# KubiakJakub01/Blokus-RL

Hardware: AMD Instinct MI355X
Metric: MCTS sims/sec on 20x20 Blokus (4 players, 256 games/GPU, 100 sims/move) (higher is better)
Workload: dtype fp32 net (fp32 operands split into f16 hi+lo, 3 f16 MFMA products, f32 accumulation: fp32-class error, tests/test_leafnet_gpu.py) / f64 search / u32 bitboards; 1 GPU; config 3 (N=1) / 4 (N=8): AlphaZero self-play 20x20, 256 concurrent games per GPU, 100 sims/move, ResNet-5x64 leaf eval; global_batch=256, parallelism=dp1 (independent games), model=resnet

## Files before the change

### blokus_rl_amd/csrc/mcts.hip

```cpp
#define BK_BOARD_SYNC() ::bk::wave_lds_sync()
#ifdef BK_STAMPS
#include <hip/hip_runtime.h>
static __device__ unsigned long long g_step_stamps[4096][16];
#define BK_MASK_STAMP(i) \
  do { if (threadIdx.x == 0 && blockIdx.x < 4096 && blockDim.x > 256) g_step_stamps[blockIdx.x][i] = __builtin_amdgcn_s_memtime(); } while (0)
#endif
#include <algorithm>
#include <cmath>
#include <cstring>
#include <vector>

#include "../../include/blokus_engine.h"
#include "ctx.h"
#include "legal_rows.h"
#include "mcts_dev.h"

namespace bk {

constexpr int kResetBlocks = 8;
__global__ __launch_bounds__(256) void k_reset(DevMcts m, const int32_t* flags) {
  const int t = blockIdx.y;
  if (flags && !flags[t]) return;
  TabEntry* tab = m.tab + (size_t)t * m.TS;
  for (int i = blockIdx.x * 256 + threadIdx.x; i < m.TS; i += kResetBlocks * 256) tab[i] = TabEntry{0ull, 0u, 0};
  if (blockIdx.x == 0 && threadIdx.x == 0) { m.tree_nodes[t] = 0; m.tree_children[t] = 0; }
}

constexpr int kSelectWaves = 4;
__global__ __launch_bounds__(64 * kSelectWaves) void k_select(DevPreset dp, DevMcts m, const uint32_t* __restrict__ roots,
                                                              const int32_t* __restrict__ active, double cpuct,
                                                              int32_t* __restrict__ status_out, float* __restrict__ obs,
                                                              uint64_t* __restrict__ mask_out, double root_eps, int t0) {
  extern __shared__ __attribute__((aligned(16))) uint32_t lds[];
  __shared__ int status_sh;
  const int t = t0 + blockIdx.x;
  const int wave = __builtin_amdgcn_readfirstlane(threadIdx.x >> 6);
  if (wave == 0) {
    const int st = select_descend(dp, m, t, roots, active, cpuct, status_out, lds, 0, nullptr, root_eps);
    if (lane_id() == 0) status_sh = st;
  }
  __syncthreads();
  select_leaf<kSelectWaves>(dp, m, t, status_sh, obs, mask_out, lds, wave);
}

constexpr int kLeafR = 1;
__global__ __launch_bounds__(256) void k_leaf_logits(DevPreset dp, DevMcts m, const float* __restrict__ feat,
                                                     int64_t ldf, int F, const float* __restrict__ W,
                                                     const float* __restrict__ bias) {
  extern __shared__ __attribute__((aligned(16))) uint32_t lds[];
  leaf_logits_tree<kLeafR>(dp, m, blockIdx.x, blockIdx.y, kLeafBlocks, feat, ldf, F, W, bias, lds);
}

__global__ __launch_bounds__(64) void k_expand_backup(DevPreset dp, DevMcts m, const float* __restrict__ logp,
                                                      const float* __restrict__ values, int prior_mode) {
  extern __shared__ __attribute__((aligned(16))) uint32_t lds[];
  expand_tree(dp, m, blockIdx.x, logp, values, prior_mode, lds);
}

__device__ __forceinline__ void wg_store_handoff() {
  __builtin_amdgcn_s_waitcnt(0x0F70);
  __syncthreads();
  asm volatile("buffer_inv sc0" ::: "memory");
}
constexpr int kStepWaves = 16;
__device__ __forceinline__ void leaf_zero_logits_tree(const DevPreset& dp, const DevMcts& m, int t,
                                                      const float* __restrict__ feat, int64_t ldf, int F,
                                                      uint32_t* lds) {
  const int K = leaf_logits_prologue(dp, m, t, 0, feat, ldf, F, lds);
  if (K < 0 || K > kLeafCap) return;
  const int32_t* ids = reinterpret_cast<const int32_t*>(lds + dp.W32pad);
  for (int j = threadIdx.x; j < K; j += blockDim.x) {
    m.leaf_ids[(size_t)t * kLeafCap + j] = ids[j];
    m.leaf_logit[(size_t)t * kLeafCap + j] = 0.0f;
  }
}
template <bool ROWS>
__device__ __forceinline__ void leaf_step_body(const DevPreset& dp, const DevMcts& m, const int t,
                                               const float* __restrict__ feat, int64_t ldf, int F,
                                               const float* __restrict__ W, const float* __restrict__ bias,
                                               const float* __restrict__ values, int do_select,
                                               const uint32_t* __restrict__ roots,
                                               const int32_t* __restrict__ active, double cpuct,
                                               int32_t* __restrict__ status_out, float* __restrict__ obs,
                                               uint64_t* __restrict__ mask_out, bool uninformed, int root_row) {
  extern __shared__ __attribute__((aligned(16))) uint32_t lds[];
  __shared__ int status_sh;
  const int wave = __builtin_amdgcn_readfirstlane(threadIdx.x >> 6);
#ifdef BK_STAMPS
#define BK_STEP_STAMP(i) \
  do { if (do_select && threadIdx.x == 0 && t < 4096) g_step_stamps[t][i] = __builtin_amdgcn_s_memtime(); } while (0)
#else
#define BK_STEP_STAMP(i) do { } while (0)
#endif
  BK_STEP_STAMP(0);
  if (ROWS && uninformed)
    leaf_zero_logits_tree(dp, m, t, feat, ldf, F, lds);
  else
    leaf_logits_tree<kLeafR>(dp, m, t, 0, 1, feat, ldf, F, W, bias, lds);
  wg_store_handoff();
  BK_STEP_STAMP(1);
  if (wave == 0) expand_tree<ROWS>(dp, m, t, nullptr, values, 2, lds);
  wg_store_handoff();
  BK_STEP_STAMP(2);
  if (!do_select) return;
  if (wave == 0) {
    const int st = select_descend<ROWS>(dp, m, t, roots, active, cpuct, status_out, lds, 0, nullptr, 1e-6, root_row);
    if (lane_id() == 0) status_sh = st;
  }
  __syncthreads();
  BK_STEP_STAMP(3);
  select_leaf<kStepWaves>(dp, m, t, status_sh, obs, mask_out, lds, wave);
  BK_STEP_STAMP(4);
#undef BK_STEP_STAMP
}
__global__ __launch_bounds__(64 * kStepWaves) void k_leaf_step(DevPreset dp, DevMcts m, const float* __restrict__ feat,
                                                                 int64_t ldf, int F, const float* __restrict__ W,
                                                                 const float* __restrict__ bias,
                                                                 const float* __restrict__ values, int do_select,
                                                                 const uint32_t* __restrict__ roots,
                                                                 const int32_t* __restrict__ active, double cpuct,
                                                                 int32_t* __restrict__ status_out,
                                                                 float* __restrict__ obs,
                                                                 uint64_t* __restrict__ mask_out, int t0) {
  leaf_step_body<false>(dp, m, t0 + blockIdx.x, feat, ldf, F, W, bias, values, do_select, roots, active, cpuct,
                        status_out, obs, mask_out, false, -1);
}

template <bool ROWS>
__device__ __forceinline__ void leaf_step_ov_body(const DevPreset& dp, const DevMcts& m, const int t,
                                                  const float* __restrict__ feat, int64_t ldf, int F,
                                                  const float* __restrict__ W, const float* __restrict__ bias,
                                                  const float* __restrict__ values, int do_select,
                                                  const uint32_t* __restrict__ roots,
                                                  const int32_t* __restrict__ active, double cpuct,
                                                  int32_t* __restrict__ status_out, float* __restrict__ obs,
                                                  uint64_t* __restrict__ mask_out, int sel_off, int skipz,
                                                  bool uninformed, int root_row) {
  extern __shared__ __attribute__((aligned(16))) uint32_t lds[];
  __shared__ int status_sh, status0_sh;
  __shared__ StepExpand sx;
  const int wave = __builtin_amdgcn_readfirstlane(threadIdx.x >> 6);
#ifdef BK_STAMPS
#define BK_OV_STAMP(i) \
  do { if (lane_id() == 0 && do_select && t < 4096) g_step_stamps[t][i] = __builtin_amdgcn_s_memtime(); } while (0)
#else
#define BK_OV_STAMP(i) do { } while (0)
#endif
  if (threadIdx.x == 0) {
    sx.ready = 0;
    sx.pready = 0;
    sx.done = 0;
    sx.leaf_ready = 0;
    sx.slice = 0;
    sx.loaded = 0;
    sx.counted = 0;
    sx.written = 0;
    sx.kready = 0;
    sx.hready = 0;
    status_sh = 0;
    status0_sh = m.leaf_status[t];
  }
  if (wave == 0) BK_OV_STAMP(0);
  LeafPre pre{0ull, 0.0f, false};
  if (wave > 0) pre = leaf_pre_load<kStepWaves - 1>(dp, m, t, feat, ldf, F);
  __syncthreads();
  const int status0 = status0_sh;
  int K = -1;
  if (wave > 0) {
    K = leaf_logits_prologue_w<kStepWaves - 1>(dp, m, t, feat, ldf, F, lds, wave, &sx, status0, &pre);
    if (wave == 1 && K >= 0) {
      wait_flag_acquire(&sx.hready);
      StepHead h;
      h.status = sx.hd_status;
      h.node = sx.hd_node;
      h.used = sx.hd_used;
      h.key = sx.hd_key;
      expand_head(m, t, h, K, &sx);
      BK_OV_STAMP(1);
    }
  }
  const int32_t* ids = reinterpret_cast<const int32_t*>(lds + dp.W32pad);
  float* lg = reinterpret_cast<float*>(lds + dp.W32pad + kLeafCap + F);
  uint32_t* lsel = lds + sel_off;
  uint32_t* m32 = lsel + kStateWords + 2 * kMaxN;
  if (wave == 0) {
    const StepHead h = backup_first<ROWS>(m, t, dp.P, values, status0);
    if (h.status == 1) {
      if (lane_id() == 0) {
        sx.hd_status = h.status;
        sx.hd_node = h.node;
        sx.hd_used = h.used;
        sx.hd_key = h.key;
        __hip_atomic_store(&sx.hready, 1, __ATOMIC_RELEASE, __HIP_MEMORY_SCOPE_WORKGROUP);
      }
    } else if (lane_id() == 0) {
      sx.err = -1;
      __hip_atomic_store(&sx.ready, 1, __ATOMIC_RELEASE, __HIP_MEMORY_SCOPE_WORKGROUP);
    }
    BK_OV_STAMP(2);
    if (do_select) {
      __builtin_amdgcn_s_waitcnt(0x0F70);
      asm volatile("buffer_inv sc0" ::: "memory");
      int* pend[3];
      pend[0] = &sx.ready;
      pend[1] = &sx.pready;
      pend[2] = &sx.err;
      const int st = select_descend<ROWS>(dp, m, t, roots, active, cpuct, status_out, lsel, h.key,
                                          h.status == 1 ? pend : nullptr, 1e-6, root_row);
      if (st == 1)
        for (int i = lane_id(); i < dp.W32pad / 4; i += kWave) reinterpret_cast<uint4*>(m32)[i] = make_uint4(0u, 0u, 0u, 0u);
      if (lane_id() == 0) {
        status_sh = st;
        __hip_atomic_store(&sx.leaf_ready, 1, __ATOMIC_RELEASE, __HIP_MEMORY_SCOPE_WORKGROUP);
      }
      BK_OV_STAMP(3);
      leaf_obs_rows<1>(dp, m, t, st, obs, lsel, lane_id());
    }
  }
  if (wave > 0 && K >= 0 && K <= kLeafCap) {
    if (ROWS && uninformed) {
      for (int j = (wave - 1) * kWave + lane_id(); j < K; j += (kStepWaves - 1) * kWave) lg[j] = 0.0f;
    } else {
      leaf_logits_dots<kLeafR>(dp, 0, K, wave - 1, kStepWaves - 1, W, bias, F, lds, nullptr, lg, skipz);
    }
    int done = 0;
    if (lane_id() == 0) done = __hip_atomic_fetch_add(&sx.done, 1, __ATOMIC_ACQ_REL, __HIP_MEMORY_SCOPE_WORKGROUP);
    done = readlane_i(done, 0);
    if (done == kStepWaves - 2) {
      BK_OV_STAMP(4);
      while (__hip_atomic_load(&sx.ready, __ATOMIC_ACQUIRE, __HIP_MEMORY_SCOPE_WORKGROUP) == 0)
        __builtin_amdgcn_s_sleep(1);
      const int err = readlane_i(sx.err, 0);
      if (err == 0) expand_children_lds(m, (int64_t)sx.off, K, ids, lg);
      BK_OV_STAMP(9);
      const bool descended = readlane_i(__hip_atomic_load(&sx.leaf_ready, __ATOMIC_RELAXED,
                                                          __HIP_MEMORY_SCOPE_WORKGROUP), 0) != 0;
      if (!descended) {
        __builtin_amdgcn_s_waitcnt(0x0F70);
        if (lane_id() == 0) __hip_atomic_store(&sx.pready, 1, __ATOMIC_RELEASE, __HIP_MEMORY_SCOPE_WORKGROUP);
      } else if (lane_id() == 0) {
        __hip_atomic_store(&sx.pready, 1, __ATOMIC_RELAXED, __HIP_MEMORY_SCOPE_WORKGROUP);
      }
      BK_OV_STAMP(5);
    }
  }
  if (do_select) {
    while (__hip_atomic_load(&sx.leaf_ready, __ATOMIC_ACQUIRE, __HIP_MEMORY_SCOPE_WORKGROUP) == 0)
      __builtin_amdgcn_s_sleep(1);
    if (readlane_i(status_sh, 0) == 1) mask_slices_claim(dp, lsel, m32, &sx.slice);
    if (wave == 0) BK_OV_STAMP(8);
  }
  __syncthreads();
  if (wave == 0) BK_OV_STAMP(6);
  if (!do_select) return;
  select_leaf<kStepWaves, true, false>(dp, m, t, status_sh, obs, mask_out, lsel, wave);
  if (wave == 0) BK_OV_STAMP(7);
#undef BK_OV_STAMP
}
__global__ __launch_bounds__(64 * kStepWaves) void k_leaf_step_ov(DevPreset dp, DevMcts m, const float* __restrict__ feat,
                                                                    int64_t ldf, int F, const float* __restrict__ W,
                                                                    const float* __restrict__ bias,
                                                                    const float* __restrict__ values, int do_select,
                                                                    const uint32_t* __restrict__ roots,
                                                                    const int32_t* __restrict__ active, double cpuct,
                                                                    int32_t* __restrict__ status_out,
                                                                    float* __restrict__ obs,
                                                                    uint64_t* __restrict__ mask_out, int sel_off,
                                                                    int skipz, int t0) {
  leaf_step_ov_body<false>(dp, m, t0 + blockIdx.x, feat, ldf, F, W, bias, values, do_select, roots, active, cpuct,
                           status_out, obs, mask_out, sel_off, skipz, false, -1);
}

struct RowTabs {
  const int32_t *tree, *net, *sims;
};
struct RowHeads {
  const float* W[BK_ARENA_MAX_NETS];
  const float* bias[BK_ARENA_MAX_NETS];
  int n;
};
__device__ __forceinline__ int row_live_tree(const RowTabs& rows, int r, int sim, int& budget) {
  const int t = __builtin_amdgcn_readfirstlane(rows.tree[r]);
  budget = 0;
  if (t < 0) return -1;
  budget = __builtin_amdgcn_readfirstlane(rows.sims[r]);
  return sim < budget ? t : -1;
}
__device__ __forceinline__ bool row_head(const RowTabs& rows, const RowHeads& hd, int r, const float*& W,
                                         const float*& bias, bool& uninformed) {
  const int k = __builtin_amdgcn_readfirstlane(rows.net[r]);
  uninformed = k < 0;
  W = k == 0 ? hd.W[0] : k == 1 ? hd.W[1] : k == 2 ? hd.W[2] : k == 3 ? hd.W[3] : nullptr;
  bias = k == 0 ? hd.bias[0] : k == 1 ? hd.bias[1] : k == 2 ? hd.bias[2] : k == 3 ? hd.bias[3] : nullptr;
  return k < hd.n;
}

__global__ __launch_bounds__(64 * kSelectWaves) void k_select_rows(DevPreset dp, DevMcts m, RowTabs rows,
                                                                   const uint32_t* __restrict__ roots, double cpuct,
                                                                   int32_t* __restrict__ status_out) {
  extern __shared__ __attribute__((aligned(16))) uint32_t lds[];
  __shared__ int status_sh;
  int budget;
  const int t = row_live_tree(rows, blockIdx.x, 0, budget);
  if (t < 0 || t >= m.T) return;
  const int wave = __builtin_amdgcn_readfirstlane(threadIdx.x >> 6);
  if (wave == 0) {
    const int st = select_descend<true>(dp, m, t, roots, nullptr, cpuct, status_out, lds, 0, nullptr, 1e-6, (int)blockIdx.x);
    if (lane_id() == 0) status_sh = st;
  }
  __syncthreads();
  select_leaf<kSelectWaves>(dp, m, t, status_sh, nullptr, nullptr, lds, wave);
}

__global__ __launch_bounds__(64 * kStepWaves) void k_leaf_step_rows(DevPreset dp, DevMcts m, RowTabs rows, int sim,
                                                                      const float* __restrict__ feat, int64_t ldf, int F,
                                                                      RowHeads heads, const float* __restrict__ values,
                                                                      int do_select, const uint32_t* __restrict__ roots,
                                                                      double cpuct, int32_t* __restrict__ status_out) {
  int budget;
  const int t = row_live_tree(rows, blockIdx.x, sim, budget);
  if (t < 0 || t >= m.T) return;
  const float *W, *bias;
  bool uninformed;
  if (!row_head(rows, heads, blockIdx.x, W, bias, uninformed)) return;
  leaf_step_body<true>(dp, m, t, feat, ldf, F, W, bias, uninformed ? nullptr : values,
                       do_select && sim + 1 < budget, roots, nullptr, cpuct, status_out, nullptr, nullptr, uninformed,
                       (int)blockIdx.x);
}

__global__ __launch_bounds__(64 * kStepWaves) void k_leaf_step_ov_rows(DevPreset dp, DevMcts m, RowTabs rows, int sim,
                                                                         const float* __restrict__ feat, int64_t ldf,
                                                                         int F, RowHeads heads,
                                                                         const float* __restrict__ values, int do_select,
                                                                         const uint32_t* __restrict__ roots, double cpuct,
                                                                         int32_t* __restrict__ status_out, int sel_off,
                                                                         int skipz) {
  int budget;
  const int t = row_live_tree(rows, blockIdx.x, sim, budget);
  if (t < 0 || t >= m.T) return;
  const float *W, *bias;
  bool uninformed;
  if (!row_head(rows, heads, blockIdx.x, W, bias, uninformed)) return;
  leaf_step_ov_body<true>(dp, m, t, feat, ldf, F, W, bias, uninformed ? nullptr : values,
                          do_select && sim + 1 < budget, roots, nullptr, cpuct, status_out, nullptr, nullptr, sel_off,
                          skipz, uninformed, (int)blockIdx.x);
}

__global__ __launch_bounds__(64) void k_arena_move(DevMcts m, RowTabs rows, const uint32_t* __restrict__ roots,
                                                   int32_t* __restrict__ action) {
  const int r = blockIdx.x, l = lane_id();
  const int t = __builtin_amdgcn_readfirstlane(rows.tree[r]);
  if (t < 0 || t >= m.T) {
    if (l == 0) action[r] = -1;
    return;
  }
  const uint64_t key = table_key(roots + (size_t)r * kStateWords);
  int64_t off;
  int K;
  if (!table_find(m, t, key, off, K, nullptr)) {
    if (l == 0) {
      action[r] = -1;
      atomicOr(&m.counters[kCtrErr], (unsigned long long)kErrMissingRoot);
    }
    return;
  }
  double best = -1.0;
  int bi = 0x7fffffff;
  for (int i = l; i < K; i += kWave) {
    const double v = (double)m.ch_N[off + i];
    if (v > best) { best = v; bi = i; }
  }
  wave_argmax(best, bi);
  if (l == 0) action[r] = K > 0 ? m.ch_id[off + bi] : -1;
}

__device__ __forceinline__ double raise_visits(uint32_t n, double e) {
  if (e == 1.0 || n <= 1u) return (double)n;
  return pow((double)n, e);
}

__global__ __launch_bounds__(64) void k_root(DevMcts m, const uint32_t* __restrict__ roots,
                                             const int32_t* __restrict__ active, double temperature, int mode,
                                             int32_t* ids, double* pi, uint32_t* n_out, double* q_out, float* p_out,
                                             int cap, int32_t* counts) {
  const int t = blockIdx.x;
  const int l = lane_id();
  if (active && !active[t]) {
    if (l == 0) counts[t] = 0;
    return;
  }
  const uint32_t* s = roots + (size_t)t * kStateWords;
  const uint64_t key = table_key(s);
  int64_t off;
  int K;
  if (!table_find(m, t, key, off, K, nullptr)) {
    if (l == 0) { counts[t] = -1; atomicOr(&m.counters[kCtrErr], (unsigned long long)kErrMissingRoot); }
    return;
  }
  if (l == 0) counts[t] = K <= cap ? K : -K;
  const int Kc = K <= cap ? K : cap;
  if (mode == 1) {
    for (int i = l; i < Kc; i += kWave) {
      ids[(size_t)t * cap + i] = m.ch_id[off + i];
      n_out[(size_t)t * cap + i] = m.ch_N[off + i];
      q_out[(size_t)t * cap + i] = m.ch_Q[off + i];
      p_out[(size_t)t * cap + i] = m.ch_P[off + i];
    }
    return;
  }
  for (int i = l; i < Kc; i += kWave) ids[(size_t)t * cap + i] = m.ch_id[off + i];
  double* o = pi + (size_t)t * cap;
  if (temperature == 0.0) {
    double best = -1.0;
    int bi = 0x7fffffff;
    for (int i = l; i < K; i += kWave) {
      const double v = (double)m.ch_N[off + i];
      if (v > best) { best = v; bi = i; }
    }
    wave_argmax(best, bi);
    for (int i = l; i < Kc; i += kWave) o[i] = i == bi ? 1.0 : 0.0;
    return;
  }
  constexpr int kRootLds = 2048;
  __shared__ double vals[kRootLds];
  __shared__ double total_sh;
  const double e = 1.0 / temperature;
  for (int i = l; i < K && i < kRootLds; i += kWave) vals[i] = raise_visits(m.ch_N[off + i], e);
  __syncthreads();
  if (l == 0) {
    double total = 0.0;
#pragma unroll 8
    for (int i = 0; i < K; ++i) total += i < kRootLds ? vals[i] : raise_visits(m.ch_N[off + i], e);
    total_sh = total;
  }
  __syncthreads();
  const double total = total_sh;
  for (int i = l; i < Kc; i += kWave) {
    const double v = i < kRootLds ? vals[i] : raise_visits(m.ch_N[off + i], e);
    o[i] = total == 0.0 ? 1.0 / (double)K : v / total;
  }
}

}

using namespace bk;

template <typename T>
static int mcts_alloc(bk_mcts* m, T** p, size_t count) {
  void* q = nullptr;
  int rc = hip_check(hipMalloc(&q, sizeof(T) * (count ? count : 1)), "hipMalloc mcts");
  if (rc) return rc;
  m->allocs.push_back(q);
  *p = (T*)q;
  return BK_OK;
}

extern "C" {

#ifdef BK_STAMPS
int bk_debug_stamps(unsigned long long* out) {
  return hip_check(hipMemcpyFromSymbol(out, HIP_SYMBOL(g_stamps), sizeof(g_stamps)), "stamps");
}
int bk_debug_mask_stamps(unsigned long long* out) {
  return hip_check(hipMemcpyFromSymbol(out, HIP_SYMBOL(g_mask_stamps), sizeof(g_mask_stamps)), "mask stamps");
}
int bk_debug_step_stamps(unsigned long long* out) {
  return hip_check(hipMemcpyFromSymbol(out, HIP_SYMBOL(g_step_stamps), sizeof(g_step_stamps)), "step stamps");
}
#endif

int bk_mcts_create(bk_ctx* ctx, int trees, int node_cap, int64_t child_cap, bk_mcts** out) {
  BK_REQUIRE(ctx && out && trees > 0 && node_cap > 0 && child_cap >= trees, "bad argument");
  BK_REQUIRE(child_cap / trees <= (int64_t)0xffffffff, "bk_mcts_create: child_cap / trees must fit 32 bits");
  BK_REQUIRE(ctx->d_items, "host-only context (created with device < 0)");
  *out = nullptr;
  bk_mcts* m = new bk_mcts();
  m->ctx = ctx;
  DevMcts& d = m->d;
  d.T = trees;
  d.node_cap = node_cap;
  int TS = 64;
  while (TS < 2 * node_cap) TS <<= 1;
  d.TS = TS;
  d.child_cap_per_tree = child_cap / trees;
  const size_t T = (size_t)trees;
  const int W64 = ctx->dp.W64;
  int rc = hip_check(hipSetDevice(ctx->device), "hipSetDevice");
  if (!rc) {
    const size_t C0 = (size_t)d.child_cap_per_tree * T;
    const size_t need = T * TS * sizeof(TabEntry) + C0 * (4 + 4 + 8 + 4) +
                        T * (kMaxDepth * 12 + kStateWords * 4 + kMaxP * 8 + W64 * 8 + kLeafCap * 8 + 64 + 64);
    size_t free_b = 0, total_b = 0;
    if (hipMemGetInfo(&free_b, &total_b) == hipSuccess && need > free_b) {
      delete m;
      char msg[256];
      snprintf(msg, sizeof msg,
               "bk_mcts_create: %d trees x node_cap %d (child_cap %lld) need %.2f GB of device memory, %.2f GB free",
               trees, node_cap, (long long)child_cap, need / 1e9, free_b / 1e9);
      bk::set_error(msg);
      return BK_ENOMEM;
    }
  }
  if (!rc) rc = mcts_alloc(m, &d.tab, T * TS);
  if (!rc) rc = mcts_alloc(m, &d.tree_nodes, T);
  if (!rc) rc = mcts_alloc(m, &d.tree_children, T);
  const size_t C = (size_t)d.child_cap_per_tree * T;
  if (!rc) rc = mcts_alloc(m, &d.ch_id, C);
  if (!rc) rc = mcts_alloc(m, &d.ch_N, C);
  if (!rc) rc = mcts_alloc(m, &d.ch_Q, C);
  if (!rc) rc = mcts_alloc(m, &d.ch_P, C);
  if (!rc) rc = mcts_alloc(m, &d.path_child, T * kMaxDepth);
  if (!rc) rc = mcts_alloc(m, &d.path_pl, T * kMaxDepth);
  if (!rc) rc = mcts_alloc(m, &d.depth, T);
  if (!rc) rc = mcts_alloc(m, &d.leaf_state, T * kStateWords);
  if (!rc) rc = mcts_alloc(m, &d.leaf_status, T);
  if (!rc) rc = mcts_alloc(m, &d.leaf_scores, T * kMaxP);
  if (!rc) rc = mcts_alloc(m, &d.leaf_mask, T * W64);
  if (!rc) rc = mcts_alloc(m, &d.leaf_ids, T * kLeafCap);
  if (!rc) rc = mcts_alloc(m, &d.leaf_logit, T * kLeafCap);
  if (!rc) rc = mcts_alloc(m, &d.leaf_K, T);
  if (!rc) rc = mcts_alloc(m, &d.counters, 8);
  if (!rc) rc = hip_check(hipMemset(d.counters, 0, 8 * sizeof(unsigned long long)), "memset counters");
  if (!rc) rc = mcts_alloc(m, &d.tree_ctr, T * 8);
  if (!rc) rc = hip_check(hipMemset(d.tree_ctr, 0, T * 8 * sizeof(unsigned long long)), "memset tree counters");
  if (!rc) rc = hip_check(hipMemset(d.leaf_status, 0, T * sizeof(int32_t)), "memset status");
  if (!rc) rc = hip_check(hipMemset(d.depth, 0, T * sizeof(int32_t)), "memset depth");
  if (rc) { bk_mcts_destroy(m); return rc; }
  rc = bk_mcts_reset(m, nullptr, nullptr);
  if (!rc) rc = hip_check(hipDeviceSynchronize(), "sync");
  if (rc) { bk_mcts_destroy(m); return rc; }
  *out = m;
  return BK_OK;
}

int bk_mcts_destroy(bk_mcts* m) {
  if (!m) return BK_OK;
  for (void* p : m->allocs) (void)hipFree(p);
  for (hipStream_t s : m->pipe_stream)
    if (s) (void)hipStreamDestroy(s);
  for (hipEvent_t e : m->pipe_step)
    if (e) (void)hipEventDestroy(e);
  for (hipEvent_t e : m->pipe_join)
    if (e) (void)hipEventDestroy(e);
  if (m->pipe_fork) (void)hipEventDestroy(m->pipe_fork);
  delete m;
  return BK_OK;
}

int bk_mcts_reset(bk_mcts* m, const int32_t* reset_flags, void* stream) {
  BK_REQUIRE(m, "null mcts");
  hipLaunchKernelGGL(k_reset, dim3(kResetBlocks, m->d.T), dim3(256), 0, (hipStream_t)stream, m->d,
                     reset_flags);
  return launch_check("k_reset");
// ... 358 lines not shown
```

### blokus_rl_amd/csrc/mcts_dev.h

```cpp
#pragma once
#include <cmath>
#include <vector>

#include "../../include/blokus_engine.h"
#include "ctx.h"
#include "legal_rows.h"

namespace bk {

constexpr int kMaxDepth = 96;
constexpr int kExpandLdsIds = 2048;
constexpr int kGatherRegs = 16;
constexpr int kLeafCap = 2048;
constexpr int kLeafBlocks = 4;
constexpr int kMaxFeat = 2048;
constexpr int kLeafQ = 16;

#ifdef BK_STAMPS
static __device__ unsigned long long g_stamps[2][4096][8];
#define BK_STAMP(k, i) \
  do { if (lane_id() == 0 && blockIdx.x < 4096) g_stamps[k][blockIdx.x][i] = __builtin_amdgcn_s_memtime(); } while (0)
#else
#define BK_STAMP(k, i) do { } while (0)
#endif
// ... 363 lines not shown
  __syncthreads();
  const int wave = threadIdx.x >> 6, l = threadIdx.x & 63;
  if (wave == 0) {
    const int K = compact_ids(dp, m32, ids, kLeafCap);
    if (l == 0) Ksh = K;
  }
  __syncthreads();
  const int K = Ksh;
  if (c == 0 && threadIdx.x == 0) {
    m.leaf_K[t] = K;
    if (K > kLeafCap) atomicOr(&m.counters[kCtrErr], (unsigned long long)kErrLeafCap);
  }
  return K;
}


__device__ __forceinline__ bool nz4(const float4& x) { return x.x != 0.f || x.y != 0.f || x.z != 0.f || x.w != 0.f; }
__device__ __forceinline__ __amdgpu_buffer_rsrc_t w_rsrc(const float* W, unsigned bytes) {
  const uintptr_t a = (uintptr_t)W;
  const uintptr_t u = ((uintptr_t)(unsigned)__builtin_amdgcn_readfirstlane((int)(a >> 32)) << 32) |
                      (unsigned)__builtin_amdgcn_readfirstlane((int)(unsigned)a);
  return __builtin_amdgcn_make_buffer_rsrc((void*)u, 0, (int)bytes, 0x00020000);
}
__device__ __forceinline__ float4 w_load(__amdgpu_buffer_rsrc_t rs, unsigned off, bool use) {
  using u32x4 = unsigned __attribute__((ext_vector_type(4)));
  const u32x4 v = __builtin_bit_cast(u32x4, __builtin_amdgcn_raw_buffer_load_b128(rs, use ? off : 0xFFFFFFF0u, 0, 0));
  return make_float4(__uint_as_float(v.x), __uint_as_float(v.y), __uint_as_float(v.z), __uint_as_float(v.w));
}
template <bool SKIP = false>
__device__ __forceinline__ float row_dot16(const float4* __restrict__ r, const float4* f4, int F4, int sub,
                                           __amdgpu_buffer_rsrc_t rs, unsigned roff) {
  float a0 = 0.f, a1 = 0.f;
  int q = sub;
  for (; q + 48 < F4; q += 64) {
    const float4 x0 = f4[q], x1 = f4[q + 16], x2 = f4[q + 32], x3 = f4[q + 48];
    float4 w0, w1, w2, w3;
    if (SKIP) {
      w0 = w_load(rs, roff + 16u * q, nz4(x0));
      w1 = w_load(rs, roff + 16u * (q + 16), nz4(x1));
      w2 = w_load(rs, roff + 16u * (q + 32), nz4(x2));
      w3 = w_load(rs, roff + 16u * (q + 48), nz4(x3));
    } else {
      w0 = r[q];
      w1 = r[q + 16];
      w2 = r[q + 32];
      w3 = r[q + 48];
    }
    a0 += w0.x * x0.x + w0.y * x0.y + w0.z * x0.z + w0.w * x0.w;
    a1 += w1.x * x1.x + w1.y * x1.y + w1.z * x1.z + w1.w * x1.w;
    a0 += w2.x * x2.x + w2.y * x2.y + w2.z * x2.z + w2.w * x2.w;
    a1 += w3.x * x3.x + w3.y * x3.y + w3.z * x3.z + w3.w * x3.w;
  }
  for (; q < F4; q += 16) {
    const float4 x0 = f4[q];
    const float4 w0 = SKIP ? w_load(rs, roff + 16u * q, nz4(x0)) : r[q];
    a0 += w0.x * x0.x + w0.y * x0.y + w0.z * x0.z + w0.w * x0.w;
  }
  float a = a0 + a1;
#pragma unroll
  for (int o = 8; o >= 1; o >>= 1) a += __shfl_xor(a, o, 16);
  return a;
}

template <int R = 1>
__device__ __forceinline__ void leaf_logits_dots(const DevPreset& dp, int lo, int hi, int wave, int nw,
                                                 const float* __restrict__ W, const float* __restrict__ bias, int F,
                                                 const uint32_t* lds, int32_t* out_ids, float* out_lg,
                                                 int skipz = 0) {
  const int32_t* ids = reinterpret_cast<const int32_t*>(lds + dp.W32pad);
  const float* f = reinterpret_cast<const float*>(lds + dp.W32pad + kLeafCap);
  const int l = threadIdx.x & 63;
  if (R > 1 && (F & 3) == 0 && F <= 64 * kLeafQ) {
    const int F4 = F >> 2;
    const float4* f4 = reinterpret_cast<const float4*>(f);
    const int sub = l & 15, quad = l >> 4;
    for (int j0 = lo + 4 * R * wave; j0 < hi; j0 += 4 * R * nw) {
      int jr[R], idr[R];
      float4 w[R][kLeafQ];
#pragma unroll
      for (int u = 0; u < R; ++u) {
        jr[u] = j0 + 4 * u + quad;
        idr[u] = ids[jr[u] < hi ? jr[u] : lo];
        const float4* r = reinterpret_cast<const float4*>(W + (size_t)idr[u] * F);
#pragma unroll
        for (int k = 0; k < kLeafQ; ++k) w[u][k] = r[sub + 16 * k < F4 ? sub + 16 * k : F4 - 1];
      }
#pragma unroll
      for (int u = 0; u < R; ++u) {
        float a0 = 0.f, a1 = 0.f;
#pragma unroll
        for (int k = 0; k < kLeafQ; ++k) {
          const int q = sub + 16 * k;
          if (q < F4) {
            const float4 x = f4[q];
            const float d = w[u][k].x * x.x + w[u][k].y * x.y + w[u][k].z * x.z + w[u][k].w * x.w;
            if ((k & 1) && sub + 16 * (k | 3) < F4)
              a1 += d;
            else
              a0 += d;
          }
        }
        float a = a0 + a1;
#pragma unroll
        for (int o = 8; o >= 1; o >>= 1) a += __shfl_xor(a, o, 16);
        if (sub == 0 && jr[u] < hi) {
          if (out_ids) out_ids[jr[u]] = idr[u];
          out_lg[jr[u]] = a + bias[idr[u]];
        }
      }
    }
  } else if ((F & 3) == 0) {
    const int F4 = F >> 2;
    const float4* f4 = reinterpret_cast<const float4*>(f);
    const int sub = l & 15, quad = l >> 4;
    const uint64_t wbytes = (uint64_t)dp.A * (uint64_t)F * 4u;
    const bool sk = skipz && wbytes < 0x7FFFFFF0ull;
    const __amdgpu_buffer_rsrc_t wrs = w_rsrc(W, sk ? (unsigned)wbytes : 0u);
    for (int j0 = lo + 4 * wave; j0 < hi; j0 += 4 * nw) {
      const int j = j0 + quad;
      const bool ok = j < hi;
      const int id = ids[ok ? j : lo];
      const float4* wr = reinterpret_cast<const float4*>(W + (size_t)id * F);
      const float a = sk ? row_dot16<true>(wr, f4, F4, sub, wrs, (unsigned)id * (unsigned)F * 4u)
                            : row_dot16<false>(wr, f4, F4, sub, wrs, 0u);
      if (sub == 0 && ok) {
        if (out_ids) out_ids[j] = id;
        out_lg[j] = a + bias[id];
      }
    }
  } else {
    for (int j = lo + wave; j < hi; j += nw) {
      const int id = ids[j];
      const float* r = W + (size_t)id * F;
      float a = 0.f;
      for (int q = l; q < F; q += kWave) a += r[q] * f[q];
      a = wave_sum_f(a);
      if (l == 0) {
        if (out_ids) out_ids[j] = id;
        out_lg[j] = a + bias[id];
      }
    }
  }
}


template <int R = 1>
__device__ __forceinline__ void leaf_logits_tree(const DevPreset& dp, const DevMcts& m, int t, int c, int nc,
                                                 const float* __restrict__ feat, int64_t ldf, int F,
                                                 const float* __restrict__ W, const float* __restrict__ bias,
                                                 uint32_t* lds) {
  const int K = leaf_logits_prologue(dp, m, t, c, feat, ldf, F, lds);
  if (K < 0 || K > kLeafCap) return;
  const int lo = (int)((int64_t)K * c / nc), hi = (int)((int64_t)K * (c + 1) / nc);
  leaf_logits_dots<R>(dp, lo, hi, (int)(threadIdx.x >> 6), (int)(blockDim.x >> 6), W, bias, F, lds,
                      m.leaf_ids + (size_t)t * kLeafCap, m.leaf_logit + (size_t)t * kLeafCap);
}

template <bool ZV = false>
__device__ __forceinline__ void expand_tree(const DevPreset& dp, const DevMcts& m, int t, const float* __restrict__ logp,
                                            const float* __restrict__ values, int prior_mode, uint32_t* lds) {
  uint32_t* m32 = lds;
  __shared__ double vsh[kMaxP];
  const int l = lane_id();
  const bool sparse = prior_mode == 2;
  const int status = m.leaf_status[t];
  const int depth = m.depth[t];
  const int node = m.tree_nodes[t];
  const int64_t used = m.tree_children[t];
  const int leafK = sparse ? m.leaf_K[t] : 0;
  const uint64_t key = table_key(m.leaf_state + (size_t)t * kStateWords);
  if (status == 0) return;
  BK_STAMP(1, 0);
  const size_t pi = (size_t)t * kMaxDepth + l;
  const bool on_path = l < depth;
  const int64_t pchild = on_path ? m.path_child[pi] : 0;
  const int ppl = on_path ? m.path_pl[pi] : 0;
  if (status == 1) {
    int err = 0;
    const int64_t room = m.child_cap_per_tree - used;
    const int64_t off = (int64_t)t * m.child_cap_per_tree + used;
    int32_t* ids_lds = reinterpret_cast<int32_t*>(m32 + dp.W32pad);
    const int cap_lds = kExpandLdsIds;
    int K;
    bool in_lds;
    BK_STAMP(1, 1);
    if (sparse) {
      K = leafK;
      in_lds = true;
      if (K > kLeafCap) err |= kErrLeafCap;
    } else {
      const uint64_t* lm = m.leaf_mask + (size_t)t * dp.W64;
      for (int j = l; j < dp.W64; j += kWave) {
        const uint64_t w = lm[j];
        m32[2 * j] = (uint32_t)w;
        m32[2 * j + 1] = (uint32_t)(w >> 32);
      }
      BK_BOARD_SYNC();
      K = compact_ids(dp, m32, ids_lds, cap_lds);
      in_lds = K <= cap_lds;
      if (!in_lds)
        K = compact_ids(dp, m32, m.ch_id + off, room > 0 ? (int)(room < 0x7fffffff ? room : 0x7fffffff) : 0);
      BK_BOARD_SYNC();
    }
    BK_STAMP(1, 2);
    if (node >= m.node_cap) err |= kErrTable;
    if (K > room) err |= kErrChildPool;
    const float* lp = sparse ? m.leaf_logit + (size_t)t * kLeafCap : logp + (size_t)t * dp.A;
    const int32_t* cid = sparse ? m.leaf_ids + (size_t)t * kLeafCap : (in_lds ? ids_lds : m.ch_id + off);
    auto logit = [&](int i) { return sparse ? lp[i] : lp[cid[i]]; };
    float x[kGatherRegs];
    int32_t xid[kGatherRegs];
#pragma unroll
    for (int j = 0; j < kGatherRegs; ++j) {
      const int i = l + j * kWave;
      const bool ok = !err && i < K;
      x[j] = ok ? logit(i) : -INFINITY;
      xid[j] = ok && in_lds ? cid[i] : 0;
    }
    int free_slot = -1;
    if (!err) {
      int64_t foff;
      int fK;
      if (table_find(m, t, key, foff, fK, &free_slot) || free_slot < 0) err |= kErrTable;
    }
    BK_STAMP(1, 3);
    if (!err) {
      float mx = -INFINITY;
#pragma unroll
      for (int j = 0; j < kGatherRegs; ++j) mx = fmaxf(mx, x[j]);
      for (int i = l + kGatherRegs * kWave; i < K; i += kWave) mx = fmaxf(mx, logit(i));
      float lse = 0.0f;
      if (prior_mode != 1) {
        mx = wave_max_f(mx);
        float sum = 0.0f;
#pragma unroll
        for (int j = 0; j < kGatherRegs; ++j) sum += l + j * kWave < K ? expf(x[j] - mx) : 0.0f;
        for (int i = l + kGatherRegs * kWave; i < K; i += kWave) sum += expf(logit(i) - mx);
        sum = wave_sum_f(sum);
        lse = logf(sum);
#pragma unroll
        for (int j = 0; j < kGatherRegs; ++j) x[j] = expf((x[j] - mx) - lse);
      }
#pragma unroll
      for (int j = 0; j < kGatherRegs; ++j) {
        const int i = l + j * kWave;
        if (i < K) {
          if (in_lds) m.ch_id[off + i] = xid[j];
          m.ch_N[off + i] = 0u;
          m.ch_Q[off + i] = 0.0;
          m.ch_P[off + i] = x[j];
        }
      }
      for (int i = l + kGatherRegs * kWave; i < K; i += kWave) {
        const float xi = logit(i);
        if (in_lds) m.ch_id[off + i] = cid[i];
        m.ch_N[off + i] = 0u;
        m.ch_Q[off + i] = 0.0;
        m.ch_P[off + i] = prior_mode != 1 ? expf((xi - mx) - lse) : xi;
      }
      if (l == 0) {
        TabEntry e;
        e.key = key;
        e.off = (uint32_t)used;
        e.K = K;
        m.tab[(size_t)t * m.TS + free_slot] = e;
        m.tree_nodes[t] = node + 1;
        m.tree_children[t] = used + K;
        ctr_add(m, t, kCtrExpanded, 1ull);
        ctr_add(m, t, kCtrLeafK, (unsigned long long)K);
      }
    } else if (l == 0) {
      atomicOr(&m.counters[kCtrErr], (unsigned long long)err);
    }
    if (l < dp.P) vsh[l] = ZV && !values ? 0.0 : (double)values[(size_t)t * dp.P + l];
  } else {
    if (l < dp.P) vsh[l] = m.leaf_scores[(size_t)t * kMaxP + l];
  }
  BK_STAMP(1, 4);
  BK_BOARD_SYNC();
  if (on_path) {
    const double v = vsh[ppl];
    const uint32_t n = m.ch_N[pchild];
    const double q = m.ch_Q[pchild];
    m.ch_Q[pchild] = ((double)n * q + v) / (double)(n + 1u);
    m.ch_N[pchild] = n + 1u;
  }
  for (int d = l + kWave; d < depth; d += kWave) {
    const size_t pd = (size_t)t * kMaxDepth + d;
    const int64_t ci = m.path_child[pd];
    const double v = vsh[m.path_pl[pd]];
    const uint32_t n = m.ch_N[ci];
    const double q = m.ch_Q[ci];
    m.ch_Q[ci] = ((double)n * q + v) / (double)(n + 1u);
    m.ch_N[ci] = n + 1u;
  }
  BK_STAMP(1, 5);
}

struct StepExpand {
  long long off;
  int K, err;
  int ready;
  int pready;
  int done;
  int leaf_ready;
  int slice;
  int loaded;
  int counted;
  int written;
  int kready;
  int hready;
  int wcnt[16];
  int hd_status, hd_node;
  long long hd_used;
  unsigned long long hd_key;
};

struct StepHead {
  int status, node;
  int64_t used;
  uint64_t key;
};
template <bool ZV = false>
__device__ __forceinline__ StepHead backup_first(const DevMcts& m, int t, int P, const float* __restrict__ values,
                                                 int status) {
  __shared__ double vsh[kMaxP];
  const int l = lane_id();
  StepHead h;
  h.status = status;
  const int depth = m.depth[t];
  h.node = m.tree_nodes[t];
  h.used = m.tree_children[t];
  h.key = table_key(m.leaf_state + (size_t)t * kStateWords);
  if (h.status == 0) return h;
  const size_t pi = (size_t)t * kMaxDepth + l;
  const bool on_path = l < depth;
  const int64_t pchild = on_path ? m.path_child[pi] : 0;
  const int ppl = on_path ? m.path_pl[pi] : 0;
  if (h.status == 1) {
    if (l < P) vsh[l] = ZV && !values ? 0.0 : (double)values[(size_t)t * P + l];
  } else {
    if (l < P) vsh[l] = m.leaf_scores[(size_t)t * kMaxP + l];
  }
  wave_lds_sync();
  if (on_path) {
    const double v = vsh[ppl];
    const uint32_t n = m.ch_N[pchild];
    const double q = m.ch_Q[pchild];
    m.ch_Q[pchild] = ((double)n * q + v) / (double)(n + 1u);
    m.ch_N[pchild] = n + 1u;
  }
  for (int d = l + kWave; d < depth; d += kWave) {
    const size_t pd = (size_t)t * kMaxDepth + d;
    const int64_t ci = m.path_child[pd];
    const double v = vsh[m.path_pl[pd]];
    const uint32_t n = m.ch_N[ci];
    const double q = m.ch_Q[ci];
    m.ch_Q[ci] = ((double)n * q + v) / (double)(n + 1u);
    m.ch_N[ci] = n + 1u;
  }
  return h;
}

__device__ __forceinline__ void expand_head(const DevMcts& m, int t, const StepHead& h, int K, StepExpand* sx) {
  const int l = lane_id();
  int err = 0;
  if (h.status == 1) {
    const int64_t room = m.child_cap_per_tree - h.used;
    if (K > kLeafCap) err |= kErrLeafCap;
    if (h.node >= m.node_cap) err |= kErrTable;
    if (K > room) err |= kErrChildPool;
    int free_slot = -1;
    if (!err) {
      int64_t foff;
      int fK;
      if (table_find(m, t, h.key, foff, fK, &free_slot) || free_slot < 0) err |= kErrTable;
    }
    if (!err) {
      if (l == 0) {
        TabEntry e;
        e.key = h.key;
        e.off = (uint32_t)h.used;
        e.K = K;
        m.tab[(size_t)t * m.TS + free_slot] = e;
        m.tree_nodes[t] = h.node + 1;
        m.tree_children[t] = h.used + K;
        ctr_add(m, t, kCtrExpanded, 1ull);
        ctr_add(m, t, kCtrLeafK, (unsigned long long)K);
      }
    } else if (l == 0) {
      atomicOr(&m.counters[kCtrErr], (unsigned long long)err);
    }
  }
  __builtin_amdgcn_s_waitcnt(0x0F70);
  if (l == 0) {
    sx->off = (long long)((int64_t)t * m.child_cap_per_tree + h.used);
    sx->K = K;
    sx->err = h.status == 1 ? err : -1;
    __hip_atomic_store(&sx->ready, 1, __ATOMIC_RELEASE, __HIP_MEMORY_SCOPE_WORKGROUP);
  }
}

struct LeafPre {
  uint64_t w;
  float f;
  bool ok;
};
template <int NW>
__device__ __forceinline__ LeafPre leaf_pre_load(const DevPreset& dp, const DevMcts& m, int t,
                                                 const float* __restrict__ feat, int64_t ldf, int F) {
  const int tid = threadIdx.x - kWave, nth = NW * kWave;
  LeafPre p;
  p.ok = dp.W64 <= nth && F <= nth;
  p.w = p.ok && tid < dp.W64 ? m.leaf_mask[(size_t)t * dp.W64 + tid] : 0ull;
  p.f = p.ok && tid < F ? feat[(size_t)t * ldf + tid] : 0.0f;
  return p;
}
template <int NW>
__device__ __forceinline__ int leaf_logits_prologue_w(const DevPreset& dp, const DevMcts& m, int t,
                                                      const float* __restrict__ feat, int64_t ldf, int F,
                                                      uint32_t* lds, int wave, StepExpand* sx, int status,
                                                      const LeafPre* pre = nullptr) {
  uint32_t* m32 = lds;
  int32_t* ids = reinterpret_cast<int32_t*>(lds + dp.W32pad);
  float* f = reinterpret_cast<float*>(lds + dp.W32pad + kLeafCap);
  if (status != 1) return -1;
  const int tid = threadIdx.x - kWave, nth = NW * kWave, l = lane_id();
  if (pre && pre->ok) {
    if (tid < dp.W64) {
      m32[2 * tid] = (uint32_t)pre->w;
      m32[2 * tid + 1] = (uint32_t)(pre->w >> 32);
    }
    if (tid < F) f[tid] = pre->f;
  } else {
    const uint64_t* lm = m.leaf_mask + (size_t)t * dp.W64;
    for (int j = tid; j < dp.W64; j += nth) {
      const uint64_t w = lm[j];
      m32[2 * j] = (uint32_t)w;
      m32[2 * j + 1] = (uint32_t)(w >> 32);
    }
    const float* ft = feat + (size_t)t * ldf;
    for (int i = tid; i < F; i += nth) f[i] = ft[i];
  }
  auto arrive_wait = [&](int* ctr) {
    if (l == 0) __hip_atomic_fetch_add(ctr, 1, __ATOMIC_ACQ_REL, __HIP_MEMORY_SCOPE_WORKGROUP);
    while (__hip_atomic_load(ctr, __ATOMIC_ACQUIRE, __HIP_MEMORY_SCOPE_WORKGROUP) < NW) __builtin_amdgcn_s_sleep(1);
  };
  arrive_wait(&sx->loaded);
  const int w = 64 * (wave - 1) + l;
  uint32_t bits = w < dp.W32 ? m32[w] : 0u;
  const int cnt = __popc(bits);
  const int incl = wave_incl_scan(cnt);
  if (l == kWave - 1) sx->wcnt[wave] = incl;
  arrive_wait(&sx->counted);
  int before = 0, K = 0;
  for (int v = 1; v <= NW; ++v) {
    const int c = sx->wcnt[v];
    before += v < wave ? c : 0;
    K += c;
  }
  int pos = before + incl - cnt;
  while (bits) {
    const int b = __ffs(bits) - 1;
    bits &= bits - 1u;
    if (pos < kLeafCap) ids[pos] = w * 32 + b;
    ++pos;
  }
  arrive_wait(&sx->written);
  if (wave == 1 && l == 0) {
    m.leaf_K[t] = K;
    if (K > kLeafCap) atomicOr(&m.counters[kCtrErr], (unsigned long long)kErrLeafCap);
    __hip_atomic_store(&sx->kready, K + 1, __ATOMIC_RELEASE, __HIP_MEMORY_SCOPE_WORKGROUP);
  }
  return K;
}

#ifdef BK_STAMPS
static __device__ unsigned long long g_mask_stamps[256][16][6];
#endif
__device__ __forceinline__ void mask_slices_claim(const DevPreset& dp, const uint32_t* s, uint32_t* m32, int* counter) {
#ifdef BK_STAMPS
  const unsigned long long t_in = __builtin_amdgcn_s_memtime();
  unsigned long long n_cl = 0, t_max = 0, t_first_claim = 0;
  int last_k = -1;
#endif
  RowCtx c = row_ctx(dp, s, (int)s[kWToMove], m32);
  for (;;) {
#ifdef BK_STAMPS
    const unsigned long long t_s = __builtin_amdgcn_s_memtime();
    if (t_first_claim == 0) t_first_claim = t_s;
#endif
#pragma unroll
    for (int d = 0; d < 5; ++d) asm volatile("" : "+v"(c.fr[d]), "+v"(c.ar[d]));
    asm volatile("" : "+v"(c.r), "+v"(c.rN1), "+v"(c.pieces));
    int k = 0;
    if (lane_id() == 0) k = __hip_atomic_fetch_add(counter, 1, __ATOMIC_RELAXED, __HIP_MEMORY_SCOPE_WORKGROUP);
    k = readlane_i(k, 0);
    if (k >= kMaskWpb) break;
    DevPreset dq = dp;
    asm volatile("" : "+s"(dq.N), "+s"(dq.num_pieces));
    orient_dispatch<kMaskWpb>(dq, c, k, std::make_index_sequence<kMaskWpb>{});
#ifdef BK_STAMPS
    ++n_cl;
    last_k = k;
    const unsigned long long d = __builtin_amdgcn_s_memtime() - t_s;
    t_max = d > t_max ? d : t_max;
#endif
  }
#ifdef BK_STAMPS
  const unsigned long long t_out = __builtin_amdgcn_s_memtime();
  unsigned long long t_warm = 0;
  if (last_k >= 0) {
    DevPreset dq = dp;
    asm volatile("" : "+s"(dq.N), "+s"(dq.num_pieces));
    const unsigned long long t0 = __builtin_amdgcn_s_memtime();
    orient_dispatch<kMaskWpb>(dq, c, last_k, std::make_index_sequence<kMaskWpb>{});
    t_warm = __builtin_amdgcn_s_memtime() - t0;
  }
  const int w = (int)(threadIdx.x >> 6);
  if (lane_id() == 0 && blockIdx.x < 256 && w < 16) {
    g_mask_stamps[blockIdx.x][w][0] = t_in;
    g_mask_stamps[blockIdx.x][w][1] = n_cl;
    g_mask_stamps[blockIdx.x][w][2] = t_out;
    g_mask_stamps[blockIdx.x][w][3] = t_max;
    g_mask_stamps[blockIdx.x][w][4] = t_warm;
    g_mask_stamps[blockIdx.x][w][5] = t_first_claim;
  }
#endif
}

__device__ __forceinline__ void expand_children_lds(const DevMcts& m, int64_t off, int K, const int32_t* ids,
                                                    const float* lg) {
  const int l = lane_id();
  float x[kGatherRegs];
  int32_t xid[kGatherRegs];
#pragma unroll
  for (int j = 0; j < kGatherRegs; ++j) {
    const int i = l + j * kWave;
    const bool ok = i < K;
    x[j] = ok ? lg[i] : -INFINITY;
    xid[j] = ok ? ids[i] : 0;
  }
  float mx = -INFINITY;
#pragma unroll
  for (int j = 0; j < kGatherRegs; ++j) mx = fmaxf(mx, x[j]);
  for (int i = l + kGatherRegs * kWave; i < K; i += kWave) mx = fmaxf(mx, lg[i]);
  mx = wave_max_f(mx);
  float sum = 0.0f;
#pragma unroll
  for (int j = 0; j < kGatherRegs; ++j) sum += l + j * kWave < K ? expf(x[j] - mx) : 0.0f;
  for (int i = l + kGatherRegs * kWave; i < K; i += kWave) sum += expf(lg[i] - mx);
  sum = wave_sum_f(sum);
  const float lse = logf(sum);
#pragma unroll
  for (int j = 0; j < kGatherRegs; ++j) x[j] = expf((x[j] - mx) - lse);
#pragma unroll
  for (int j = 0; j < kGatherRegs; ++j) {
    const int i = l + j * kWave;
    if (i < K) {
      m.ch_id[off + i] = xid[j];
      m.ch_N[off + i] = 0u;
      m.ch_Q[off + i] = 0.0;
      m.ch_P[off + i] = x[j];
    }
  }
  for (int i = l + kGatherRegs * kWave; i < K; i += kWave) {
    m.ch_id[off + i] = ids[i];
    m.ch_N[off + i] = 0u;
    m.ch_Q[off + i] = 0.0;
    m.ch_P[off + i] = expf((lg[i] - mx) - lse);
  }
}

}

struct bk_mcts {
  bk_ctx* ctx = nullptr;
  bk::DevMcts d{};
  std::vector<void*> allocs;
  static constexpr int kMaxGroups = 4;
  bool pipe_ready = false;
  hipStream_t pipe_stream[kMaxGroups - 1] = {};
  hipEvent_t pipe_fork = nullptr, pipe_step[kMaxGroups] = {}, pipe_join[kMaxGroups - 1] = {};
};
```

Baseline: 1.465 million sims/s.

## Split child expansion stores across waves via work-claiming shares

The last wave to finish the logit dot products now computes only the softmax max and log-sum-exp. The child-node stores are then cut into wave-sized shares that any idle wave can claim through an LDS atomic counter, including waves spinning on leaf_ready or on a bounded spin loop. This spreads the global-memory writes that one wave used to do alone. The prologue also keeps each thread's 32-bit mask word in a register instead of staging it through LDS with a barrier, and mask_slices_claim is skipped when all slices are already claimed. The cost is more atomics and added synchronisation complexity.

```diff
diff --git a/blokus_rl_amd/csrc/mcts.hip b/blokus_rl_amd/csrc/mcts.hip
--- a/blokus_rl_amd/csrc/mcts.hip
+++ b/blokus_rl_amd/csrc/mcts.hip
@@ -149,6 +149,9 @@
   if (threadIdx.x == 0) {
     sx.ready = 0;
     sx.pready = 0;
+    sx.sready = 0;
+    sx.sclaim = 0;
+    sx.sstored = 0;
     sx.done = 0;
     sx.leaf_ready = 0;
     sx.slice = 0;
@@ -157,6 +160,9 @@
     sx.written = 0;
     sx.kready = 0;
     sx.hready = 0;
+#ifdef BK_STAMPS
+    sx.stamp = do_select && t < 4096;
+#endif
     status_sh = 0;
     status0_sh = m.leaf_status[t];
   }
@@ -217,10 +223,47 @@
       leaf_obs_rows<1>(dp, m, t, st, obs, lsel, lane_id());
     }
   }
+  auto children_shares = [&]() {
+    const int ns = readlane_i(sx.nshare, 0);
+    const int64_t off = (int64_t)sx.off;
+    const float mx = sx.mx, lse = sx.lse;
+    const bool descended = readlane_i(__hip_atomic_load(&sx.leaf_ready, __ATOMIC_RELAXED,
+                                                        __HIP_MEMORY_SCOPE_WORKGROUP), 0) != 0;
+    auto claim = [&]() {
+      int c = 0;
+      if (lane_id() == 0) c = __hip_atomic_fetch_add(&sx.sclaim, 1, __ATOMIC_RELAXED, __HIP_MEMORY_SCOPE_WORKGROUP);
+      return c;
+    };
+    int n = 0, c = claim(), cn = claim();
+    c = readlane_i(c, 0);
+    while (c < ns) {
+      store_children_share(m, off, K, ids, lg, mx, lse, c);
+      ++n;
+      c = readlane_i(cn, 0);
+      if (c < ns) cn = claim();
+    }
+    if (n == 0) return;
+    int prev = 0;
+    if (!descended) {
+      __builtin_amdgcn_s_waitcnt(0x0F70);
+      if (lane_id() == 0) prev = __hip_atomic_fetch_add(&sx.sstored, n, __ATOMIC_ACQ_REL, __HIP_MEMORY_SCOPE_WORKGROUP);
+    } else if (lane_id() == 0) {
+      prev = __hip_atomic_fetch_add(&sx.sstored, n, __ATOMIC_RELAXED, __HIP_MEMORY_SCOPE_WORKGROUP);
+    }
+    if (readlane_i(prev, 0) + n == ns) {
+      if (lane_id() == 0)
+        __hip_atomic_store(&sx.pready, 1, descended ? __ATOMIC_RELAXED : __ATOMIC_RELEASE, __HIP_MEMORY_SCOPE_WORKGROUP);
+      BK_OV_STAMP(5);
+    }
+  };
+  constexpr int kShareSpins = 64;
+  bool share = false;
   if (wave > 0 && K >= 0 && K <= kLeafCap) {
     if (ROWS && uninformed) {
       for (int j = (wave - 1) * kWave + lane_id(); j < K; j += (kStepWaves - 1) * kWave) lg[j] = 0.0f;
     } else {
+      if (wave == 2) BK_OV_STAMP(13);
+      if (wave == 1) BK_OV_STAMP(14);
       leaf_logits_dots<kLeafR>(dp, 0, K, wave - 1, kStepWaves - 1, W, bias, F, lds, nullptr, lg, skipz);
     }
     int done = 0;
@@ -228,27 +271,49 @@
     done = readlane_i(done, 0);
     if (done == kStepWaves - 2) {
       BK_OV_STAMP(4);
+#ifdef BK_STAMPS
+      if (lane_id() == 0 && do_select && t < 4096) g_step_stamps[t][15] = (unsigned long long)wave;
+#endif
       while (__hip_atomic_load(&sx.ready, __ATOMIC_ACQUIRE, __HIP_MEMORY_SCOPE_WORKGROUP) == 0)
         __builtin_amdgcn_s_sleep(1);
       const int err = readlane_i(sx.err, 0);
-      if (err == 0) expand_children_lds(m, (int64_t)sx.off, K, ids, lg);
+      float mx = 0.0f, lse = 0.0f;
+      if (err == 0) softmax_stats_lds(K, lg, mx, lse);
+      if (lane_id() == 0) {
+        sx.mx = mx;
+        sx.lse = lse;
+        sx.nshare = err == 0 ? (K + kWave - 1) / kWave : 0;
+        __hip_atomic_store(&sx.sready, 1, __ATOMIC_RELEASE, __HIP_MEMORY_SCOPE_WORKGROUP);
+      }
       BK_OV_STAMP(9);
-      const bool descended = readlane_i(__hip_atomic_load(&sx.leaf_ready, __ATOMIC_RELAXED,
-                                                          __HIP_MEMORY_SCOPE_WORKGROUP), 0) != 0;
-      if (!descended) {
-        __builtin_amdgcn_s_waitcnt(0x0F70);
+      if (err != 0 || K == 0) {
         if (lane_id() == 0) __hip_atomic_store(&sx.pready, 1, __ATOMIC_RELEASE, __HIP_MEMORY_SCOPE_WORKGROUP);
-      } else if (lane_id() == 0) {
-        __hip_atomic_store(&sx.pready, 1, __ATOMIC_RELAXED, __HIP_MEMORY_SCOPE_WORKGROUP);
+        BK_OV_STAMP(5);
+      } else {
+        children_shares();
       }
-      BK_OV_STAMP(5);
+    } else {
+      share = true;
     }
   }
   if (do_select) {
-    while (__hip_atomic_load(&sx.leaf_ready, __ATOMIC_ACQUIRE, __HIP_MEMORY_SCOPE_WORKGROUP) == 0)
+    while (__hip_atomic_load(&sx.leaf_ready, __ATOMIC_ACQUIRE, __HIP_MEMORY_SCOPE_WORKGROUP) == 0) {
+      if (share && __hip_atomic_load(&sx.sready, __ATOMIC_ACQUIRE, __HIP_MEMORY_SCOPE_WORKGROUP) != 0) {
+        children_shares();
+        share = false;
+      } else {
+        __builtin_amdgcn_s_sleep(1);
+      }
+    }
+    if (readlane_i(status_sh, 0) == 1 &&
+        readlane_i(__hip_atomic_load(&sx.slice, __ATOMIC_RELAXED, __HIP_MEMORY_SCOPE_WORKGROUP), 0) < kMaskWpb)
+      mask_slices_claim(dp, lsel, m32, &sx.slice);
+    if (wave == 0) BK_OV_STAMP(8);
+  }
+  if (share) {
+    for (int n = 0; n < kShareSpins && __hip_atomic_load(&sx.sready, __ATOMIC_ACQUIRE, __HIP_MEMORY_SCOPE_WORKGROUP) == 0; ++n)
       __builtin_amdgcn_s_sleep(1);
-    if (readlane_i(status_sh, 0) == 1) mask_slices_claim(dp, lsel, m32, &sx.slice);
-    if (wave == 0) BK_OV_STAMP(8);
+    if (__hip_atomic_load(&sx.sready, __ATOMIC_ACQUIRE, __HIP_MEMORY_SCOPE_WORKGROUP) != 0) children_shares();
   }
   __syncthreads();
   if (wave == 0) BK_OV_STAMP(6);
diff --git a/blokus_rl_amd/csrc/mcts_dev.h b/blokus_rl_amd/csrc/mcts_dev.h
--- a/blokus_rl_amd/csrc/mcts_dev.h
+++ b/blokus_rl_amd/csrc/mcts_dev.h
@@ -689,6 +689,11 @@
   int K, err;
   int ready;
   int pready;
+  float mx, lse;
+  int sready;
+  int nshare;
+  int sclaim;
+  int sstored;
   int done;
   int leaf_ready;
   int slice;
@@ -701,6 +706,9 @@
   int hd_status, hd_node;
   long long hd_used;
   unsigned long long hd_key;
+#ifdef BK_STAMPS
+  int stamp;
+#endif
 };
 
 struct StepHead {
@@ -789,7 +797,7 @@
 }
 
 struct LeafPre {
-  uint64_t w;
+  uint32_t w;
   float f;
   bool ok;
 };
@@ -798,8 +806,8 @@
                                                  const float* __restrict__ feat, int64_t ldf, int F) {
   const int tid = threadIdx.x - kWave, nth = NW * kWave;
   LeafPre p;
-  p.ok = dp.W64 <= nth && F <= nth;
-  p.w = p.ok && tid < dp.W64 ? m.leaf_mask[(size_t)t * dp.W64 + tid] : 0ull;
+  p.ok = dp.W32 <= nth && F <= nth;
+  p.w = p.ok && tid >= 0 && tid < dp.W32 ? reinterpret_cast<const uint32_t*>(m.leaf_mask + (size_t)t * dp.W64)[tid] : 0u;
   p.f = p.ok && tid < F ? feat[(size_t)t * ldf + tid] : 0.0f;
   return p;
 }
@@ -813,11 +821,8 @@
   float* f = reinterpret_cast<float*>(lds + dp.W32pad + kLeafCap);
   if (status != 1) return -1;
   const int tid = threadIdx.x - kWave, nth = NW * kWave, l = lane_id();
-  if (pre && pre->ok) {
-    if (tid < dp.W64) {
-      m32[2 * tid] = (uint32_t)pre->w;
-      m32[2 * tid + 1] = (uint32_t)(pre->w >> 32);
-    }
+  const bool own = pre && pre->ok;
+  if (own) {
     if (tid < F) f[tid] = pre->f;
   } else {
     const uint64_t* lm = m.leaf_mask + (size_t)t * dp.W64;
@@ -833,13 +838,21 @@
     if (l == 0) __hip_atomic_fetch_add(ctr, 1, __ATOMIC_ACQ_REL, __HIP_MEMORY_SCOPE_WORKGROUP);
     while (__hip_atomic_load(ctr, __ATOMIC_ACQUIRE, __HIP_MEMORY_SCOPE_WORKGROUP) < NW) __builtin_amdgcn_s_sleep(1);
   };
-  arrive_wait(&sx->loaded);
+#ifdef BK_STAMPS
+#define BK_PRO_STAMP(i) \
+  do { if (wave == 2 && l == 0 && sx->stamp) g_step_stamps[t][i] = __builtin_amdgcn_s_memtime(); } while (0)
+#else
+#define BK_PRO_STAMP(i) do { } while (0)
+#endif
+  if (!own) arrive_wait(&sx->loaded);
+  BK_PRO_STAMP(10);
   const int w = 64 * (wave - 1) + l;
-  uint32_t bits = w < dp.W32 ? m32[w] : 0u;
+  uint32_t bits = own ? pre->w : w < dp.W32 ? m32[w] : 0u;
   const int cnt = __popc(bits);
   const int incl = wave_incl_scan(cnt);
   if (l == kWave - 1) sx->wcnt[wave] = incl;
   arrive_wait(&sx->counted);
+  BK_PRO_STAMP(11);
   int before = 0, K = 0;
   for (int v = 1; v <= NW; ++v) {
     const int c = sx->wcnt[v];
@@ -854,6 +867,8 @@
     ++pos;
   }
   arrive_wait(&sx->written);
+  BK_PRO_STAMP(12);
+#undef BK_PRO_STAMP
   if (wave == 1 && l == 0) {
     m.leaf_K[t] = K;
     if (K > kLeafCap) atomicOr(&m.counters[kCtrErr], (unsigned long long)kErrLeafCap);
@@ -916,42 +931,37 @@
 #endif
 }
 
-__device__ __forceinline__ void expand_children_lds(const DevMcts& m, int64_t off, int K, const int32_t* ids,
-                                                    const float* lg) {
+__device__ __forceinline__ void softmax_stats_lds(int K, const float* lg, float& mx_out, float& lse_out) {
   const int l = lane_id();
-  float x[kGatherRegs];
-  int32_t xid[kGatherRegs];
-#pragma unroll
-  for (int j = 0; j < kGatherRegs; ++j) {
-    const int i = l + j * kWave;
-    const bool ok = i < K;
-    x[j] = ok ? lg[i] : -INFINITY;
-    xid[j] = ok ? ids[i] : 0;
-  }
   float mx = -INFINITY;
-#pragma unroll
-  for (int j = 0; j < kGatherRegs; ++j) mx = fmaxf(mx, x[j]);
-  for (int i = l + kGatherRegs * kWave; i < K; i += kWave) mx = fmaxf(mx, lg[i]);
+#pragma nounroll
+  for (int i = l; i < K; i += 4 * kWave) {
+    float x[4];
+#pragma unroll
+    for (int u = 0; u < 4; ++u) x[u] = i + u * kWave < K ? lg[i + u * kWave] : -INFINITY;
+#pragma unroll
+    for (int u = 0; u < 4; ++u) mx = fmaxf(mx, x[u]);
+  }
   mx = wave_max_f(mx);
   float sum = 0.0f;
-#pragma unroll
-  for (int j = 0; j < kGatherRegs; ++j) sum += l + j * kWave < K ? expf(x[j] - mx) : 0.0f;
-  for (int i = l + kGatherRegs * kWave; i < K; i += kWave) sum += expf(lg[i] - mx);
+#pragma nounroll
+  for (int i = l; i < K; i += 4 * kWave) {
+    float x[4];
+#pragma unroll
+    for (int u = 0; u < 4; ++u) x[u] = i + u * kWave < K ? lg[i + u * kWave] : -INFINITY;
+#pragma unroll
+    for (int u = 0; u < 4; ++u) x[u] = i + u * kWave < K ? expf(x[u] - mx) : 0.0f;
+#pragma unroll
+    for (int u = 0; u < 4; ++u) sum += x[u];
+  }
   sum = wave_sum_f(sum);
-  const float lse = logf(sum);
-#pragma unroll
-  for (int j = 0; j < kGatherRegs; ++j) x[j] = expf((x[j] - mx) - lse);
-#pragma unroll
-  for (int j = 0; j < kGatherRegs; ++j) {
-    const int i = l + j * kWave;
-    if (i < K) {
-      m.ch_id[off + i] = xid[j];
-      m.ch_N[off + i] = 0u;
-      m.ch_Q[off + i] = 0.0;
-      m.ch_P[off + i] = x[j];
-    }
-  }
-  for (int i = l + kGatherRegs * kWave; i < K; i += kWave) {
+  mx_out = mx;
+  lse_out = logf(sum);
+}
+__device__ __forceinline__ void store_children_share(const DevMcts& m, int64_t off, int K, const int32_t* ids,
+                                                     const float* lg, float mx, float lse, int c) {
+  const int i = c * kWave + lane_id();
+  if (i < K) {
     m.ch_id[off + i] = ids[i];
     m.ch_N[off + i] = 0u;
     m.ch_Q[off + i] = 0.0;
```

After: 1.472 million sims/s (median of 6 runs). Within noise of the previous version (+0.5%).
